# DomhnallBoyle/lip2speech-unit

Hardware: AMD Instinct MI355X
Metric: real-time factor (audio-sec/wall-sec), end-to-end lip->16kHz audio, 4s@25fps clips (higher is better)
Workload: dtype fp16; 1 GPU; e2e lip->units->wav (BASELINE configs[3]: AV-HuBERT large 24L + conformer 12x512 + multi_input HiFi-GAN), 4-s 100-frame 88x88 clips, batch 640 per GPU; clips_per_gpu=640, streams=1, clips_per_launch=640, frames_per_clip=100, hipgraph=True, input=uint8 96x96 frames resident in HBM, crop+normalise on device, enc_layers=24, conf_layers=12, parallelism=clip-parallel dp1

## Files before the change

include/lip2speech_hip.h:

```cpp
#ifndef LIP2SPEECH_HIP_H
#define LIP2SPEECH_HIP_H

#include <stddef.h>
#include <stdint.h>

#ifdef __cplusplus
extern "C" {
#endif

#define L2S_ABI_VERSION 16

enum { L2S_F16 = 0, L2S_BF16 = 1, L2S_F32 = 2 };

enum { L2S_OK = 0, L2S_EINVAL = -1, L2S_ESHAPE = -2, L2S_EALIGN = -3, L2S_EUNSUPPORTED = -4 };

enum {
  L2S_ACT_NONE = 0,
  L2S_ACT_RELU = 1,
  L2S_ACT_GELU = 2,
  L2S_ACT_SWISH = 3,
  L2S_ACT_PRELU = 4,
  L2S_ACT_LRELU = 5,
  L2S_ACT_TANH = 6
};
// ... 123 lines not shown
                              int B, int T, int C, int dtype, void* stream);
int l2s_lens_from_mask(const uint8_t* mask, int32_t* lens, int B, int T, void* stream);
int l2s_split_hi_lo(const float* x, int ldx, void* hi, void* lo, int ld16, int act, float slope, const int32_t* lens,
                    int len_mul, int B, int T, int C, int dtype, void* stream);

typedef struct l2s_respair_desc {
  const void* X; const void* W1; const void* W2; const float* b1; const float* b2;
  void* Y; float* XS; const int32_t* lens;
  int32_t len_mul, B, T, C, k, dil, last, accumulate, dtype;
  float slope;
} l2s_respair_desc;
int l2s_respair(const l2s_respair_desc* d, void* stream);
int l2s_respair_variant(const l2s_respair_desc* d);

typedef struct l2s_respair_final_desc {
  const void* X[3]; const void* W1[3]; const void* W2[3]; const float* b1[3]; const float* b2[3];
  int32_t k[3], dil[3];
  void* Y; const int32_t* lens;
  int32_t n, len_mul, B, T, C, dtype;
  float slope;
} l2s_respair_final_desc;
int l2s_respair_final(const l2s_respair_final_desc* d, void* stream);

int l2s_basicblock_fused(const void* x, const void* w1, const float* b1, const float* s1, const void* w2, const float* b2,
                         const float* s2, void* y, int n_images, int H, int W, int C, int dtype, void* stream);
int l2s_basiclayer_fused(const void* x, const void* const* w, const float* const* bias, const float* const* slope, int n_blocks,
                         void* y, int n_images, int H, int W, int C, int dtype, void* stream);
#define L2S_BB_PADDED64 576064
#define L2S_BB_PHASE64 512064
#define L2S_BB_PHASE128 256128
int l2s_basicblock_variant(int n_images, int H, int W, int C, int n_blocks, int dtype);
int l2s_basicstage128_tail_fused(const void* x0, const void* t0, const void* wa, const float* ba, const float* sa, const void* w1,
                                 const float* b1, const float* s1, const void* w2, const float* b2, const float* s2, void* y,
                                 int n_images, int H, int W, int dtype, void* stream);

int l2s_conv_post_tanh(const float* x, const float* w, float bias, float* wav, int16_t* pcm, const int32_t* lens,
                       int len_mul, int B, int T, int C, int k, void* stream);

int l2s_resblock_fused(const void* xl, const void* w, const float* bias, float* xs, void* xl_out,
                       const int32_t* lens, int len_mul, int B, int T, int C, int k, int d0, int d1, int d2,
                       int accumulate, float slope, int dtype, void* stream);

int l2s_resstage_fused(const void* xl, const void* const* w, const float* const* bias, const int* ks, const int* dils,
                       int n_blocks, float* xs, void* xl_out, const int32_t* lens, int len_mul, int B, int T, int C,
                       float slope, int xs_final, int dtype, void* stream);

// ... 106 lines not shown
```

lip2speech_unit_amd/_lib.py:

```python
import ctypes
import os

_HERE = os.path.dirname(os.path.abspath(__file__))
LIB_PATH = os.environ.get("L2S_LIB_PATH") or os.path.join(_HERE, "liblip2speech_hip.so")

F16, BF16, F32 = 0, 1, 2
ACT_NONE, ACT_RELU, ACT_GELU, ACT_SWISH, ACT_PRELU, ACT_LRELU, ACT_TANH = range(7)
F_RES_PRE, F_RES_POST, F_ACCUM, F_DUAL, F_MASK, F_OUT_F32, F_RES_F32 = (1 << i for i in range(7))
MODE_LINEAR, MODE_CONV1D, MODE_CONV2D = 0, 1, 2
ABI_VERSION = 16
SEQ_VARIANT_F32, LN_GENERIC, ATTN_RESIDENT = 2000, 10, 1000
BB_PADDED64, BB_PHASE64, BB_PHASE128 = 576064, 512064, 256128

_ERR = {-1: "L2S_EINVAL", -2: "L2S_ESHAPE", -3: "L2S_EALIGN", -4: "L2S_EUNSUPPORTED"}


class L2SError(RuntimeError):
    pass


class GemmDesc(ctypes.Structure):
    _fields_ = [
        ("A", ctypes.c_void_p), ("W", ctypes.c_void_p), ("C", ctypes.c_void_p), ("C2", ctypes.c_void_p),
        ("bias", ctypes.c_void_p), ("slope", ctypes.c_void_p), ("R", ctypes.c_void_p), ("lens", ctypes.c_void_p),
# ... 13 lines not shown
        ("ktab", ctypes.c_void_p),
    ]


_vp, _i, _f = ctypes.c_void_p, ctypes.c_int, ctypes.c_float


class RespairDesc(ctypes.Structure):
    _fields_ = [("X", ctypes.c_void_p), ("W1", ctypes.c_void_p), ("W2", ctypes.c_void_p), ("b1", ctypes.c_void_p),
                ("b2", ctypes.c_void_p), ("Y", ctypes.c_void_p), ("XS", ctypes.c_void_p), ("lens", ctypes.c_void_p),
                ("len_mul", ctypes.c_int32), ("B", ctypes.c_int32), ("T", ctypes.c_int32), ("C", ctypes.c_int32),
                ("k", ctypes.c_int32), ("dil", ctypes.c_int32), ("last", ctypes.c_int32), ("accumulate", ctypes.c_int32),
                ("dtype", ctypes.c_int32), ("slope", ctypes.c_float)]


class RespairFinalDesc(ctypes.Structure):
    _fields_ = [("X", ctypes.c_void_p * 3), ("W1", ctypes.c_void_p * 3), ("W2", ctypes.c_void_p * 3), ("b1", ctypes.c_void_p * 3),
                ("b2", ctypes.c_void_p * 3), ("k", ctypes.c_int32 * 3), ("dil", ctypes.c_int32 * 3),
                ("Y", ctypes.c_void_p), ("lens", ctypes.c_void_p),
                ("n", ctypes.c_int32), ("len_mul", ctypes.c_int32), ("B", ctypes.c_int32), ("T", ctypes.c_int32),
                ("C", ctypes.c_int32), ("dtype", ctypes.c_int32), ("slope", ctypes.c_float)]


SIGNATURES = {
    "l2s_abi_version": ([], ctypes.c_int),
    "l2s_build_info": ([], ctypes.c_char_p),
    "l2s_tapgemm": ([ctypes.POINTER(GemmDesc), _vp], _i),
    "l2s_tapgemm_variant": ([ctypes.POINTER(GemmDesc)], _i),
    "l2s_tapgemm_epilogue_family": ([ctypes.POINTER(GemmDesc)], _i),
    "l2s_stem_conv3d": ([_vp, _i, _vp, _vp, _vp, _vp, _i, _i, _i, _i, _i, _vp], _i),
    "l2s_stem_pool_fused": ([_vp, _i, _vp, _vp, _vp, _vp, _i, _i, _i, _i, _i, _vp], _i),
    "l2s_stem_pool_fused_u8": ([_vp, _i, _i, _i, _f, _f, _vp, _vp, _vp, _vp, _i, _i, _i, _vp], _i),
    "l2s_maxpool2d_3x3s2": ([_vp, _vp, _i, _i, _i, _i, _i, _vp], _i),
    "l2s_avgpool_hw": ([_vp, _vp, _i, _i, _i, _i, _vp], _i),
    "l2s_layernorm": ([_vp, _i, _i, _vp, _vp, _f, _vp, _i, _i, _vp, _i, _i, _i, _i, _vp, _i, _i, _i, _vp], _i),
    "l2s_layernorm_variant": ([_vp, _i, _i, _vp, _vp, _vp, _i, _i, _vp, _i, _i, _i, _i, _vp, _i, _i, _i], _i),
    "l2s_attention_variant": ([_vp, _i, _vp, _i, _vp, _i, _vp, _vp, _vp, _i, _i, _i, _i, _i], _i),
    "l2s_glu_dwconv_tile": ([_i, _i, _i, _i, _i], _i),
    "l2s_attention": ([_vp, _i, _vp, _i, _vp, _i, _vp, _vp, _vp, _i, _i, _i, _i, _i, _vp], _i),
    "l2s_glu_dwconv_swish": ([_vp, _vp, _vp, _vp, _vp, _i, _i, _i, _i, _i, _i, _vp], _i),
    "l2s_greedy_decode": ([_vp, _i, _vp, _i, _i, _i, _i, _f, _f, _vp, _vp, _vp, _vp], _i),
    "l2s_beam_decode": ([_vp, _i, _vp, _i, _i, _i, _i, _f, _f, _i, _vp, ctypes.c_size_t, _vp, _vp, _vp, _vp, _vp], _i),
    "l2s_beam_decode_workspace": ([_i, _i, _i], ctypes.c_size_t),
    "l2s_ctc_frames": ([_vp, _i, _vp, _i, _i, _i, _i, _i, _vp, _vp, _vp, _vp], _i),
    "l2s_ctc_beam_search": ([_vp, _vp, _vp, _i, _i, _i, _i, _i, _i, _vp, ctypes.c_size_t, _vp, _vp, _vp, _vp], _i),
    "l2s_ctc_beam_workspace": ([_i, _i, _i], ctypes.c_size_t),
# ... 1 lines not shown
    "l2s_repeat2_cast": ([_vp, _vp, _i, _i, _i, _i, _vp], _i),
    "l2s_splitk_reduce": ([_vp, _i, _i, _vp, _i, _i, _i, _vp], _i),
    "l2s_splitk_reduce_layernorm": ([_vp, _i, _i, _vp, _i, _vp, _vp, _f, _vp, _i, _i, _i, _i, _vp, _i, _i, _i, _vp], _i),
    "l2s_cast_f32_to_16": ([_vp, _i, _vp, _i, _i, _i, _i, _vp], _i),
    "l2s_cast_16_to_f32": ([_vp, _i, _vp, _i, _i, _i, _i, _vp], _i),
    "l2s_broadcast_rows": ([_vp, _i, _vp, _i, _i, _vp, _i, _i, _i, _i, _i, _i, _vp], _i),
    "l2s_transpose_ct_to_tc": ([_vp, _vp, _i, _i, _vp, _i, _i, _i, _i, _i, _vp], _i),
    "l2s_embedding": ([_vp, _vp, _vp, _i, _vp, _i, _i, _i, _i, _vp], _i),
    "l2s_embedding_tokens": ([_vp, _i, _i, _vp, _i, _vp, _i, _vp, _i, _i, _i, _i, _i, _vp], _i),
    "l2s_rows_f32_to_16_masked": ([_vp, _i, _vp, _i, _i, _vp, _i, _i, _i, _i, _i, _vp], _i),
    "l2s_lens_from_mask": ([_vp, _vp, _i, _i, _vp], _i),
    "l2s_basicblock_fused": ([_vp, _vp, _vp, _vp, _vp, _vp, _vp, _vp, _i, _i, _i, _i, _i, _vp], _i),
    "l2s_basiclayer_fused": ([_vp, _vp, _vp, _vp, _i, _vp, _i, _i, _i, _i, _i, _vp], _i),
    "l2s_basicblock_variant": ([_i, _i, _i, _i, _i, _i], _i),
    "l2s_stem_pool_frames": ([_i, _i], _i),
    "l2s_basicstage128_tail_fused": ([_vp] * 12 + [_i, _i, _i, _i, _vp], _i),
    "l2s_split_hi_lo": ([_vp, _i, _vp, _vp, _i, _i, _f, _vp, _i, _i, _i, _i, _i, _vp], _i),
    "l2s_conv_post_tanh": ([_vp, _vp, _f, _vp, _vp, _vp, _i, _i, _i, _i, _i, _vp], _i),
    "l2s_resblock_fused": ([_vp, _vp, _vp, _vp, _vp, _vp, _i, _i, _i, _i, _i, _i, _i, _i, _i, _f, _i, _vp], _i),
    "l2s_resstage_fused": ([_vp, _vp, _vp, _vp, _vp, _i, _vp, _vp, _vp, _i, _i, _i, _i, _f, _i, _i, _vp], _i),
    "l2s_respair": ([ctypes.POINTER(RespairDesc), _vp], _i),
    "l2s_respair_variant": ([ctypes.POINTER(RespairDesc)], _i),
    "l2s_respair_final": ([ctypes.POINTER(RespairFinalDesc), _vp], _i),
    "l2s_preprocess_frames": ([_vp, _vp, _i, _i, _i, _i, _i, _f, _f, _i, _vp], _i),
    "l2s_mel_spectrogram": ([_vp, _i, ctypes.c_int64, _vp, _i, _i, _vp, _vp, _vp, _vp, _i, _i, _i, _i, _i, _f, _vp], _i),
    "l2s_stft_mel": ([_vp, _i, ctypes.c_int64, _vp, _i, _i, _vp, _vp, _vp, _vp, _i, _i, _i, _i, _i, _i, _f, _f, _vp], _i),
    "l2s_unit_ce": ([_vp, _i, _vp, _i, _vp, _i, _i, _i, _i, _i, _i, _vp, _vp, _vp, _vp, _vp], _i),
    "l2s_mel_l1_sc": ([_vp, _i, _vp, _i, _vp, _i, _i, _i, _i, _vp, _vp, _vp, _vp, _vp], _i),
    "l2s_ctc_loss_workspace": ([_i, _i, _i], ctypes.c_size_t),
    "l2s_ctc_loss": ([_vp, _i, _vp, _i, _i, _i, _i, _i, _vp, _vp, _vp, _i, _vp, ctypes.c_size_t, _vp, _vp], _i),
    "l2s_wave_stem_workspace": ([_i, _i], ctypes.c_size_t),
    "l2s_wave_stem": ([_vp, _i, ctypes.c_int64, _vp, _i, _i, _vp, _vp, _vp, _f, _vp, _i, _i, _i, _vp, ctypes.c_size_t, _i, _vp], _i),
    "l2s_kmeans_assign": ([_vp, _i, _vp, _vp, _vp, _i, _i, _i, _i, _i, _vp, _vp, _vp], _i),
    "l2s_kmeans_nearest_workspace": ([_i], ctypes.c_size_t),
    "l2s_kmeans_nearest": ([_vp, _i, ctypes.c_int64, _vp, _i, _vp, _vp, _i, _i, _vp, _vp, _vp, _vp, ctypes.c_size_t, _vp], _i),
    "l2s_kmeans_update_workspace": ([_i, _i], ctypes.c_size_t),
    "l2s_kmeans_update": ([_vp, _i, ctypes.c_int64, _vp, _i, _vp, _vp, _vp, _i, _i, _vp, _vp, _vp, _vp, ctypes.c_size_t, _vp], _i),
    "l2s_kmeans_pp_workspace": ([_i], ctypes.c_size_t),
    "l2s_kmeans_pp_pot": ([_vp, _i, ctypes.c_int64, _vp, _i, _i, _vp, _i, _vp, _vp, _vp, _vp, _vp, _vp, ctypes.c_size_t, _vp], _i),
    "l2s_kmeans_pp_pick": ([_vp, _i, _vp, _i, _vp, _vp, _vp, _vp], _i),
    "l2s_stoi_resample": ([_vp, _i, ctypes.c_int64, _vp, _i, _i, _vp, _vp, ctypes.c_int64, _i, _vp], _i),
    "l2s_stoi_frames": ([_vp, ctypes.c_int64, _vp, _i, _i, _vp, _vp, _i, _vp, _vp], _i),
    "l2s_stoi_bands": ([_vp, _vp, ctypes.c_int64, _vp, _i, _i, _vp, _i, _vp, _vp, _vp, _vp, _vp, _i, _vp], _i),
    "l2s_stoi_scores": ([_vp, _i, _vp, _i, _vp, _i, _vp, _vp, _vp, _vp], _i),
    "l2s_wav_gain": ([_vp, _i, ctypes.c_int64, _vp, _i, _i, _f, _vp, _vp], _i),
    "l2s_stft_mel_power": ([_vp, _i, ctypes.c_int64, _vp, _vp, _vp, _i, _i, _vp, _vp, _vp, _vp, _i, _i, _i, _i, _i, _i, _vp], _i),
# ... 51 lines not shown
```

lip2speech_unit_amd/csrc/respair_phase.hip:

```cpp
#include "phase_stream.h"
#include "respair_args.h"
#include <cstdlib>

using namespace l2s;
using l2s_rp::RpArgs;

int l2s_respair_grid(int ntiles, int slots);

namespace {

constexpr int XT1 = 8;
constexpr int XRQ = 4;
template <int CH>
struct XGeo {
  static constexpr int NWC = CH / 64, NWR = 8 / NWC, NBLK = CH / 64;
  static constexpr int RM = NWR * 64;
  static constexpr int RPR = RM + 56;
  static constexpr int BLK_B = RPR * 128;
  static constexpr int REGION = NBLK * BLK_B;
  static constexpr int QROWS = NWC * 32;
  static constexpr int Q_B = QROWS * 128;
  static constexpr int DPW = QROWS >= 64 ? QROWS / 64 : 1;
  static constexpr int RPS = DPW * 8;
  static constexpr int BIAS_OFF = REGION + XRQ * Q_B;
// ... 166 lines not shown
    for (int i = 0; i < MI; ++i)
#pragma unroll
      for (int h = 0; h < 2; ++h) {
        const u32x4_t q = resp[i][h];
        const uint32_t w4[4] = {q.x, q.y, q.z, q.w};
#pragma unroll
        for (int e = 0; e < 8; ++e) {
          const float r = ET::to_f32((uint16_t)((w4[e >> 1] >> ((e & 1) * 16)) & 0xffff));
          acc[i][2 * h + (e >> 2)][e & 3] += fminf(r, r * inv_slope);
        }
      }
  }
  __device__ __forceinline__ void add_res(Acc& acc, const u32x2_t (&resq)[MI][NI], float inv_slope) const {
#pragma unroll
    for (int i = 0; i < MI; ++i)
#pragma unroll
      for (int j = 0; j < NI; ++j) {
        const float r[4] = {ET::to_f32((uint16_t)(resq[i][j].x & 0xffff)), ET::to_f32((uint16_t)(resq[i][j].x >> 16)),
                            ET::to_f32((uint16_t)(resq[i][j].y & 0xffff)), ET::to_f32((uint16_t)(resq[i][j].y >> 16))};
#pragma unroll
        for (int e = 0; e < 4; ++e) acc[i][j][e] += fminf(r[e], r[e] * inv_slope);
      }
  }
  __device__ __forceinline__ void write_t1(const Acc& acc, int g0, int len, float slope) const {
    u32x2_t t1v[MI][NI];
#pragma unroll
    for (int i = 0; i < MI; ++i) {
      const int t = g0 + wr * 64 + i * 16 + lm;
      const uint32_t km = (unsigned)t < (unsigned)len ? 0xffffffffu : 0u;
#pragma unroll
      for (int j = 0; j < NI; ++j) {
        f32x4_t v = acc[i][j];
        const f32x4_t sc = v * slope;
#pragma unroll
        for (int e = 0; e < 4; ++e) v[e] = fmaxf(v[e], sc[e]);
        t1v[i][j].x = ET::pack2(v[0], v[1]) & km;
        t1v[i][j].y = ET::pack2(v[2], v[3]) & km;
      }
    }
    __builtin_amdgcn_s_barrier();
    asm volatile("" ::: "memory");
#pragma unroll
    for (int i = 0; i < MI; ++i) {
      const int R = wr * 64 + i * 16 + lm + XT1;
      const uint32_t ta = lds_base + (uint32_t)wc * G::BLK_B + (uint32_t)R * 128;
      if constexpr (PAIRED) {
#pragma unroll
        for (int h = 0; h < 2; ++h)
          lds_write_u4(ta + (uint32_t)(((4 * h + lg) ^ (R & 7)) << 4),
                       u32x4_t{t1v[i][2 * h].x, t1v[i][2 * h].y, t1v[i][2 * h + 1].x, t1v[i][2 * h + 1].y});
      } else {
#pragma unroll
        for (int j = 0; j < NI; ++j) lds_write_u2(ta + (uint32_t)(((2 * j + (lg >> 1)) ^ (R & 7)) << 4) + (uint32_t)((lg & 1) * 8), t1v[i][j]);
      }
    }
  }
  __device__ __forceinline__ static int64_t out_row(int r, int unit, int g0, int halo, int T) {
    const int t = g0 + r;
    return (r >= halo && r < G::RM - halo && t < T) ? (int64_t)unit * T + t : (int64_t)-1;
  }
  __device__ __forceinline__ void store_y(uint16_t* Y, Acc& acc, int unit, int g0, int halo, int T, int len, float slope) const {
    auto rowmap = [&](int r) -> int64_t { return out_row(r, unit, g0, halo, T); };
    l2s_gemm_desc p = {};
    p.C = Y; p.bias = nullptr; p.N = CH; p.ldc = CH; p.act = L2S_ACT_LRELU; p.act_slope = slope; p.alpha = 1.f;
    p.mask_T = T; p.mask_mul = 1;
    int ln = lane;
    asm volatile("" : "+v"(ln));
    epilogue_direct16<ET, MI, NI, L2S_EPI_F16 + 3, decltype(rowmap), NoHook, true>(p, acc, ln, wr * 64, wc * 64, 0, rowmap, unit * T, len);
  }
};

template <typename ET, int CH, int KIND>
__global__ __launch_bounds__(512) void respair_phase_kernel(const RpArgs a) {
  using G = XGeo<CH>;
  constexpr int MI = 4, NI = 4;
  constexpr bool PAIRED = KIND == 0;
  extern __shared__ __attribute__((aligned(16))) uint16_t lds[];
  const int tid = threadIdx.x;
  const TileWalk tiles(a.ntiles, a.xcd_order);
// ... 203 lines not shown
      pc.barrier_then_stagger();
      pc.template run_conv<0>(acc1, k, dil, h2, stage_one);

      pc.level();
      {
        u32x4_t resp[MI][2];
        pc.read_res(resp, h1);
        pc.add_res(sum, resp, inv_slope);
      }
      pc.write_t1(acc1, g0, len, slope);
      asm volatile("s_waitcnt lgkmcnt(0)" ::: "memory");
      pc.barrier_then_stagger();
      pc.template run_conv<1>(sum, k, dil, h2, stage_one);

      pc.level();
      if (j + 1 < nj) issue_patch(c_i, j + 1);
      else if (c_i + 1 < tiles.n) issue_patch(c_i + 1, 0);
    }
    pc.store_y(a.Y, sum, unit, g0, h2max, T, len, slope);
  }
  wait_vmcnt<0>();
}

template <typename ET, int CH>
int launch_respair_final(const l2s_rp::RpFinalArgs& a, hipStream_t st) {
  using G = XGeo<CH>;
  constexpr int SMEM = G::BIAS_OFF + 4 * CH * 4;
  static_assert(SMEM <= 160 * 1024, "LDS");
  auto kern = respair_final_kernel<ET, CH>;
  static L2sSmemOptIn opt_in;
  if (int e = l2s_smem_opt_in(kern, SMEM, opt_in)) return e;
  const int grid = l2s_respair_grid(a.ntiles, 256);
  hipLaunchKernelGGL(kern, dim3(grid), dim3(512), SMEM, st, a);
  L2S_CHECK_LAUNCH();
  return L2S_OK;
}

template <typename ET, int CH, int KIND>
int launch_respair_phase(const RpArgs& a, hipStream_t st) {
  using G = XGeo<CH>;
  auto kern = respair_phase_kernel<ET, CH, KIND>;
  static L2sSmemOptIn opt_in;
  if (int e = l2s_smem_opt_in(kern, G::SMEM, opt_in)) return e;
  const int grid = l2s_respair_grid(a.ntiles, 256);
  hipLaunchKernelGGL(kern, dim3(grid), dim3(512), G::SMEM, st, a);
  L2S_CHECK_LAUNCH();
// ... 44 lines not shown
    a.X[j] = (const uint16_t*)d->X[j]; a.W1[j] = (const uint16_t*)d->W1[j]; a.W2[j] = (const uint16_t*)d->W2[j];
    a.b1[j] = d->b1[j]; a.b2[j] = d->b2[j]; a.k[j] = d->k[j]; a.dil[j] = d->dil[j];
    h2max = h2 > h2max ? h2 : h2max;
  }
  for (int j = d->n; j < 3; ++j) { a.X[j] = a.X[0]; a.W1[j] = a.W1[0]; a.W2[j] = a.W2[0]; a.b1[j] = a.b1[0]; a.b2[j] = a.b2[0]; a.k[j] = a.k[0]; a.dil[j] = a.dil[0]; }
  if ((uintptr_t)d->Y & 15) return L2S_EALIGN;
  a.Y = (uint16_t*)d->Y; a.lens = d->lens; a.nj = d->n; a.len_mul = d->len_mul; a.T = d->T; a.h2max = h2max;
  a.S = l2s_respair_phase_rows(d->C) - 2 * h2max;
  a.tiles_per_clip = (d->T + a.S - 1) / a.S;
  a.ntiles = d->B * a.tiles_per_clip;
  a.xcd_order = 1;
  a.slope = d->slope;
  hipStream_t st = (hipStream_t)stream;
  auto go = [&](auto et) -> int {
    using ET = decltype(et);
    if (d->C == 256) return launch_respair_final<ET, 256>(a, st);
    if (d->C == 128) return launch_respair_final<ET, 128>(a, st);
    return launch_respair_final<ET, 64>(a, st);
  };
  if (d->dtype == L2S_F16) return go(ElemF16{});
  if (d->dtype == L2S_BF16) return go(ElemBF16{});
  return L2S_EINVAL;
}
```

lip2speech_unit_amd/ops.py:

```python
import ctypes
import os
from typing import Optional

import torch

from . import _lib
from ._lib import (ACT_GELU, ACT_LRELU, ACT_NONE, ACT_PRELU, ACT_RELU, ACT_SWISH, ACT_TANH, BF16, F16, F32, F_ACCUM,
                   F_DUAL, F_MASK, F_OUT_F32, F_RES_F32, F_RES_POST, F_RES_PRE, MODE_CONV1D, MODE_CONV2D,
                   MODE_LINEAR, GemmDesc, L2SError, check)

_TORCH16 = {F16: torch.float16, BF16: torch.bfloat16, F32: torch.float32}
_DTYPE_NAME = {F16: "f16", BF16: "bf16", F32: "f32"}


class KernelProfiler:

    def __init__(self, detail=False):
        self.records = []
        self.detail = detail

    def summary(self):
        torch.cuda.synchronize()
        agg = {}
        for key, fl, by, e0, e1, shape in self.records:
# ... 442 lines not shown
    d.lens = fake if lens else None
    d.len_mul, d.B, d.T, d.C, d.k, d.dil = len_mul, B, T, C, k, dil
    d.last, d.accumulate, d.dtype, d.slope = last, int(bool(accumulate)), dtype, float(slope)
    return _lib.load().l2s_respair_variant(ctypes.byref(d))


def respair_final(xs_l, w1s, b1s, w2s, b2s, y, *, B, T, C, ks, dils, slope, lens=None, len_mul=1, dtype=F16):
    lib = _lib.load()
    n = len(xs_l)
    if not (1 <= n <= 3 and len(w1s) == len(w2s) == len(b1s) == len(b2s) == len(ks) == len(dils) == n):
        raise L2SError("respair_final: 1..3 ResBlocks, one entry per list each")
    d = _lib.RespairFinalDesc()
    for j in range(n):
        d.X[j], d.W1[j], d.W2[j] = _ptr(_req(xs_l[j], _TORCH16[dtype], "x_l")), _ptr(w1s[j]), _ptr(w2s[j])
        d.b1[j], d.b2[j] = _ptr(_req(b1s[j], torch.float32, "b1")), _ptr(_req(b2s[j], torch.float32, "b2"))
        d.k[j], d.dil[j] = int(ks[j]), int(dils[j])
    if lens is not None and lens.dtype != torch.int32:
        raise L2SError("lens must be int32")
    d.Y, d.lens = _ptr(_req(y, _TORCH16[dtype], "y")), _ptr(lens)
    d.n, d.len_mul, d.B, d.T, d.C, d.dtype, d.slope = n, len_mul, B, T, C, dtype, float(slope)
    _run(f"l2s_respair_final<C{C}>", lambda: lib.l2s_respair_final(ctypes.byref(d), _stream()),
         flops=sum(2.0 * B * T * C * C * k * 2 for k in ks), nbytes=float(B) * T * C * 2 * (n + 1) + sum(2.0 * 2 * C * C * k for k in ks),
         shape=f"M{B * T} n{n}")


def preprocess_frames(frames, y, *, B, T, Hin, Win, crop=88, mean=0.421, std=0.165, dtype=F16):
    _run("l2s_preprocess_frames", lambda: _lib.load().l2s_preprocess_frames(_ptr(frames), _ptr(y), B, T, Hin, Win, crop, mean, std, dtype, _stream()))


def mel_spectrogram(wav, mel, basis, fb, fb_range, *, B, S, T_rows, n_samples=None, ldw=None, ldm=None, n_fft=640, hop=160, n_mels=80,
                    floor=1e-5):
    if wav.dtype not in (torch.float32, torch.int16):
        raise L2SError(f"wav: expected float32 or int16, got {wav.dtype}")
    if n_samples is not None and n_samples.dtype != torch.int32:
        raise L2SError("n_samples must be int32")
    _req(wav, None, "wav"), _req(mel, torch.float32, "mel"), _req(basis, torch.float32, "basis"), _req(fb, torch.float32, "fb")
    _req(fb_range, torch.int32, "fb_range")
    frames = float(B) * T_rows
    _run("l2s_mel_spectrogram", lambda: _lib.load().l2s_mel_spectrogram(
        _ptr(wav), int(wav.dtype == torch.int16), ldw if ldw is not None else S, _ptr(n_samples), B, S, _ptr(basis), _ptr(fb),
        _ptr(fb_range), _ptr(mel), ldm if ldm is not None else n_mels, T_rows, n_fft, hop, n_mels, float(floor), _stream()),
        flops=2.0 * frames * n_fft * n_fft, nbytes=float(B) * S * wav.element_size() + 4.0 * frames * n_mels + 4.0 * n_fft * n_fft)


def stft_mel(wav, mel, basis, fb, fb_range, *, B, S, T_rows, n_fft, hop, pad, mag_eps=0.0, n_samples=None, ldw=None, ldm=None, n_mels=80,
             floor=1e-5):
# ... 752 lines not shown
                      "int len_mul=1, int dtype=0) -> ()",
    "transpose_ct_to_tc": "(Tensor x, Tensor(a!) y, *, int B, int C, int T, int ldy, int col0=0, Tensor? lens=None, int len_mul=1, "
                          "int dtype=0) -> ()",
    "embedding": "(Tensor code, Tensor table, Tensor(a!) y, *, int B, int L, int C, int? ldy=None, Tensor? lens=None, int dtype=0) -> ()",
    "embedding_tokens": "(Tensor tok, Tensor table, Tensor(a!) y, *, int B, int L, int C, int token_offset=4, int? ldt=None, "
                        "int? ldy=None, Tensor? lens=None, int len_mul=1, int dtype=0) -> ()",
    "rows_f32_to_16_masked": "(Tensor x, Tensor(a!) y, *, int B, int T, int C, int? ldx=None, int? ldy=None, int col0=0, "
                             "Tensor? lens=None, int len_mul=1, int dtype=0) -> ()",
    "lens_from_mask": "(Tensor? padding_mask, int B, int T, Device device) -> Tensor",
    "basicblock_fused": "(Tensor x, Tensor w1, Tensor b1, Tensor s1, Tensor w2, Tensor b2, Tensor s2, Tensor(a!) y, *, int n_images, "
                        "int H, int W, int C=64, int dtype=0) -> ()",
    "basiclayer_fused": _BL,
    "basicstage128_tail_fused": "(Tensor x0, Tensor t0, Tensor wa, Tensor ba, Tensor sa, Tensor w1, Tensor b1, Tensor s1, Tensor w2, "
                                "Tensor b2, Tensor s2, Tensor(a!) y, *, int n_images, int H, int W, int dtype=0) -> ()",
    "split_hi_lo": "(Tensor x, Tensor(a!) hi, Tensor(b!) lo, *, int B, int T, int C, int act=0, float slope=0.0, int? ldx=None, "
                   "int? ld16=None, Tensor? lens=None, int len_mul=1, int dtype=0) -> ()",
    "conv_post_tanh": _CPT,
    "resblock_fused": "(Tensor xl, Tensor w, Tensor bias, Tensor(a!) xs, Tensor(b!)? xl_out, *, int B, int T, int C, int k, int[] dil, "
                      "bool accumulate, float slope, Tensor? lens=None, int len_mul=1, int dtype=0) -> ()",
    "resstage_fused": "(Tensor xl, Tensor[] ws, Tensor[] biases, Tensor(a!) xs, Tensor(b!)? xl_out, *, int B, int T, int C, int[] ks, "
                      "int[] dils, float slope, Tensor? lens=None, int len_mul=1, int dtype=0, bool xs_final=True) -> ()",
    "respair": _RP,
    "respair_final": "(Tensor[] xs_l, Tensor[] w1s, Tensor[] b1s, Tensor[] w2s, Tensor[] b2s, Tensor(a!) y, *, int B, int T, int C, int[] ks, "
                     "int[] dils, float slope, Tensor? lens=None, int len_mul=1, int dtype=0) -> ()",
    "preprocess_frames": "(Tensor frames, Tensor(a!) y, *, int B, int T, int Hin, int Win, int crop=88, float mean=0.421, "
                         "float std=0.165, int dtype=0) -> ()",
    "mel_spectrogram": "(Tensor wav, Tensor(a!) mel, Tensor basis, Tensor fb, Tensor fb_range, *, int B, int S, int T_rows, "
                       "Tensor? n_samples=None, int? ldw=None, int? ldm=None, int n_fft=640, int hop=160, int n_mels=80, "
                       "float floor=1e-05) -> ()",
    "stft_mel": "(Tensor wav, Tensor(a!) mel, Tensor basis, Tensor fb, Tensor fb_range, *, int B, int S, int T_rows, int n_fft, int hop, "
                "int pad, float mag_eps=0.0, Tensor? n_samples=None, int? ldw=None, int? ldm=None, int n_mels=80, "
                "float floor=1e-05) -> ()",
    "unit_ce": "(Tensor logits, Tensor target, Tensor(a!) nll, Tensor(b!) smooth, Tensor(c!) n_correct, Tensor(d!) n_tok, *, int B, "
               "int T2, int V, int? ldl=None, int? ldt=None, Tensor? lens=None, int len_mul=2, int pad_idx=1, "
               "int ignore_prefix=0) -> ()",
    "mel_l1_sc": "(Tensor pred, Tensor targ, Tensor(a!) l1, Tensor(b!) sq, Tensor(c!) tsq, Tensor(d!) n_rows, *, int B, int Tm_pred, "
                 "int Tm_targ, int crop_len, Tensor? lens=None, int len_mul=4, int n_mels=80) -> ()",
    "ctc_loss": "(Tensor logits, Tensor targets, Tensor tgt_lens, Tensor tgt_offs, Tensor(a!) workspace, Tensor(b!) nll, *, int B, "
                "int L, int V, int S_max, int blank=0, int? ldl=None, Tensor? lens=None, int len_mul=2) -> ()",
    "wave_stem": "(Tensor wav, Tensor w, Tensor gamma, Tensor beta, Tensor(a!) workspace, Tensor(b!) out, *, int B, int S, int T_rows, "
                 "int C=512, Tensor? n_samples=None, int? ldw=None, int? ldo=None, float eps=1e-05, int dtype=0) -> ()",
    "kmeans_assign": "(Tensor x, Tensor centers, Tensor cnorm, Tensor(a!) ids, *, int B, int T, int D, int K, int? ldx=None, "
                     "Tensor? lens=None, int len_mul=1, Tensor(b!)? best2=None) -> ()",
    "kmeans_nearest": "(Tensor x, Tensor centers, Tensor cnorm, *, int M, int D, int K, Tensor? rows=None, Tensor(a!)? ids=None, "
                      "Tensor(b!)? dmin=None, Tensor(c!)? inertia=None, Tensor(d!)? workspace=None, int? ldx=None) -> ()",
    "kmeans_update": "(Tensor x, Tensor ids, Tensor centers, Tensor counts, Tensor(a!) centers_out, Tensor(b!) counts_out, "
# ... 32 lines not shown
                    "Tensor? suppress=None, Tensor? begin_suppress=None, Tensor? step=None, int first_step=0, "
                    "Tensor(d!)? logits=None, int? ldx=None, int? lde=None, int dtype=0) -> ()",
    "whisper_advance": "(Tensor(a!) token, Tensor logprob, Tensor(b!) tokens, Tensor(c!) sum_logprob, Tensor(d!) lengths, "
                       "Tensor(e!) done, Tensor tok_emb, Tensor pos_emb, Tensor(f!) x_next, Tensor(g!) pos, Tensor(h!) n_active, *, "
                       "int B, int V, int d, int eot, int? lde=None, int? ldx=None, int dtype=0) -> ()",
    "beam_attention": "(Tensor q, Tensor(a!) k_cache, Tensor(b!) v_cache, Tensor(c!) out, *, int B, int beam, int H, int hd, "
                      "Tensor? k_new=None, Tensor? v_new=None, Tensor? anc=None, Tensor? step=None, Tensor? enc_lens=None, "
                      "Tensor? n_live=None, Tensor? finished=None, int? ldq=None, int? ld_new=None, int? ldo=None, int dtype=0) -> ()",
    "beam_select": "(Tensor logits, Tensor scores, Tensor step, Tensor max_len, Tensor(a!) cand_score, Tensor(b!) cand_slot, "
                   "Tensor(c!) cand_token, *, int B, int beam, int V, int pad, int unk, int eos, int min_len=1, float temperature=1.0, "
                   "float unk_penalty=0.0, Tensor? n_live=None, Tensor? finished=None, int? ldl=None) -> ()",
    "beam_advance": "(Tensor cand_score, Tensor cand_slot, Tensor cand_token, Tensor(a!) tokens, Tensor(b!) anc, Tensor(c!) scores, "
                    "Tensor(d!) n_live, Tensor(e!) finished, Tensor(f!) parents, Tensor(g!) hyp_tokens, Tensor(h!) hyp_len, "
                    "Tensor(i!) hyp_score, Tensor(j!) nhyp, Tensor(k!) out_tokens, Tensor(l!) out_len, Tensor(m!) out_score, "
                    "Tensor max_len, Tensor emb, Tensor pos_table, Tensor(n!) x_next, Tensor(o!) step, Tensor(p!) n_active, *, int B, "
                    "int beam, int V, int d, int eos, int pad, float embed_scale=1.0, float lenpen=1.0, bool normalize_scores=True, "
                    "int? lde=None, int? ldx=None, int dtype=0) -> ()",
    "logfbank": "(Tensor wav, Tensor(a!) out, Tensor basis, Tensor fb, Tensor fb_range, *, int B, int S, int T_rows, int stack=4, "
                "bool normalize=True, Tensor? n_samples=None, Tensor? n_rows=None, int? ldw=None, int? ldo=None) -> ()",
}
ENTRY_OF = {n: "l2s_" + n for n in _SCHEMAS}
ENTRY_OF.update({"maxpool2d_3x3s2": "l2s_maxpool2d_3x3s2", "avgpool_hw": "l2s_avgpool_hw"})
HOST_QUERIES = ("l2s_abi_version", "l2s_build_info", "l2s_tapgemm_variant", "l2s_tapgemm_epilogue_family", "l2s_attention_variant", "l2s_layernorm_variant", "l2s_respair_variant",
                "l2s_glu_dwconv_tile", "l2s_basicblock_variant", "l2s_stem_pool_frames", "l2s_beam_decode_workspace",
                "l2s_ctc_beam_workspace", "l2s_ctc_loss_workspace", "l2s_wave_stem_workspace", "l2s_kmeans_nearest_workspace",
                "l2s_kmeans_update_workspace", "l2s_kmeans_pp_workspace", "l2s_vocab_argmax_workspace", "l2s_whisper_logmel_workspace",
                "l2s_beam_select_workspace")
ALIASES = {"frontend3d_stem": "stem_pool_fused", "resnet_trunk": "basiclayer_fused", "linear_epilogue": "tapgemm",
           "posconv_gelu": "tapgemm", "convtranspose1d": "tapgemm", "mel_head": "tapgemm", "mhsa_padmask": "attention",
           "relpos_mhsa": "attention", "conformer_conv_module": "glu_dwconv_swish", "greedy_unit_decode": "greedy_decode",
           "resblock1": "respair", "tanh_to_int16": "conv_post_tanh"}

_TORCH_LIB = torch.library.Library("lip2speech", "DEF")


def _fake_none(*a, **k):
    return None


def _fake_beam_decode(logits, *, B, T2, V, beam, ldl=None, lens=None, len_mul=1, temperature=1.0, lenpen=1.0):
    return (logits.new_empty((B, beam, T2 + 1), dtype=torch.int32), logits.new_empty((B, beam, T2 + 1), dtype=torch.float32),
            logits.new_empty((B, beam), dtype=torch.float32), logits.new_empty((B,), dtype=torch.int32))


def _fake_lens_from_mask(padding_mask, B, T, device):
    return torch.empty(B, device=device, dtype=torch.int32)
# ... 52 lines not shown
```

lip2speech_unit_amd/vocoder.py:

```python
import os

import torch
import torch.nn as nn

from . import ops
from .ops import ACT_GELU, ACT_LRELU, F_ACCUM, F_DUAL, F_MASK, F_RES_POST, MODE_CONV1D
from .packing import PackedState, convtranspose_fused, convtranspose_phases, pack_conv1d

LRELU_SLOPE = 0.1
FUSED_PAIR = os.environ.get("L2S_RESPAIR", "1") != "0"
FUSED_PAIR256 = os.environ.get("L2S_RESPAIR256", "1") != "0"
PAIR_MIN_TILES = int(os.environ.get("L2S_RESPAIR_MIN_TILES", "64"))
PAIR_ROWS = {256: 128, 128: 256, 64: 512}
FUSED_UPS = os.environ.get("L2S_FUSED_UPS", "1") != "0"
FUSED_UPS_MAX_CIN = int(os.environ.get("L2S_FUSED_UPS_MAX_CIN", "128"))
FUSED_STAGE = os.environ.get("L2S_RESSTAGE", "1") != "0"
FUSED_FINAL = os.environ.get("L2S_RESPAIR_FINAL", "1") != "0"
SKIP_DEAD_XS = os.environ.get("L2S_SKIP_DEAD_XS", "1") != "0"


class AttrDict(dict):

    def __init__(self, *args, **kwargs):
        super().__init__(*args, **kwargs)
        self.__dict__ = self


def get_padding(kernel_size, dilation=1):
    return int((kernel_size * dilation - dilation) / 2)


class _WN(nn.Module):

    def __init__(self, shape, bias_n, g_dim0):
        super().__init__()
        self.weight_g = nn.Parameter(torch.ones(g_dim0, 1, 1))
        self.weight_v = nn.Parameter(torch.zeros(*shape))
        self.bias = nn.Parameter(torch.zeros(bias_n))

    def effective_weight(self):
        if hasattr(self, "weight") and isinstance(getattr(self, "weight"), torch.Tensor):
# ... 197 lines not shown
                            act_slope=LRELU_SLOPE, lens=lens, mask_T=T // fd, mask_mul=mul // u // fd, flags=F_MASK, dtype=dt)
            elif pair_stage or fused_stage:
                x = None
                for ph in st["phases"]:
                    ops.tapgemm(x_l, ph["w"], xl, M=M_in, N=C, Cin=st["cin"], ntaps=ph["ntaps"], mode=MODE_CONV1D, T_out=T,
                                T_in=T, stride=1, dil=-1, off=ph["off"], out_row_mul=u, out_row_add=ph["r"], bias=st["b"],
                                act=ACT_LRELU, act_slope=LRELU_SLOPE, lens=lens, mask_T=To, mask_mul=mul, flags=F_MASK,
                                dtype=dt)
            else:
                x = torch.empty(M, C, device=dev, dtype=t16)
                for ph in st["phases"]:
                    ops.tapgemm(x_l, ph["w"], x, M=M_in, N=C, Cin=st["cin"], ntaps=ph["ntaps"], mode=MODE_CONV1D, T_out=T,
                                T_in=T, stride=1, dil=-1, off=ph["off"], out_row_mul=u, out_row_add=ph["r"], bias=st["b"],
                                C2=xl, ldc2=C, lens=lens, mask_T=To, mask_mul=mul, flags=F_DUAL | F_MASK,
                                slope2=LRELU_SLOPE, dtype=dt)
            nxt = torch.empty(M, C, device=dev, dtype=t16)
            last_stage = si == len(P["stages"]) - 1
            final_fused = pair_stage and FUSED_FINAL and SKIP_DEAD_XS and not last_stage and len(st["rbs"]) <= 3
            xs = None if final_fused else torch.empty(M, C, device=dev, dtype=torch.float32)
            if pair_stage:
                finals = []
                for j, rb in enumerate(st["rbs"]):
                    cur_l = xl
                    for m, cv in enumerate(rb["convs"]):
                        if final_fused and m == len(rb["convs"]) - 1:
                            finals.append((cur_l, cv, rb["k"]))
                        elif m < len(rb["convs"]) - 1:
                            ol = torch.empty(M, C, device=dev, dtype=t16)
                            ops.respair(cur_l, cv["w1"], cv["b1"], cv["w2"], cv["b2"], B=B, T=To, C=C, k=rb["k"], dil=cv["d"],
                                        slope=LRELU_SLOPE, y=ol, lens=lens, len_mul=mul, dtype=dt)
                            cur_l = ol
                        else:
                            dual = (j == len(st["rbs"]) - 1) and not last_stage
                            ops.respair(cur_l, cv["w1"], cv["b1"], cv["w2"], cv["b2"], B=B, T=To, C=C, k=rb["k"], dil=cv["d"],
                                        slope=LRELU_SLOPE, xs=xs, y=nxt if dual else None, accumulate=j > 0, lens=lens,
                                        len_mul=mul, dtype=dt, xs_final=not (dual and SKIP_DEAD_XS))
                if finals:
                    ops.respair_final([f[0] for f in finals], [f[1]["w1"] for f in finals], [f[1]["b1"] for f in finals],
                                      [f[1]["w2"] for f in finals], [f[1]["b2"] for f in finals], nxt, B=B, T=To, C=C,
                                      ks=[f[2] for f in finals], dils=[f[1]["d"] for f in finals], slope=LRELU_SLOPE, lens=lens,
                                      len_mul=mul, dtype=dt)
                x_l, T = nxt, To
                continue
            if fused_stage:
                if FUSED_STAGE and [rb["k"] for rb in st["rbs"]] == [3, 7, 11]:
                    ops.resstage_fused(xl, [rb["fw"] for rb in st["rbs"]], [rb["fb"] for rb in st["rbs"]], xs,
                                       None if last_stage else nxt, B=B, T=To, C=C, ks=[rb["k"] for rb in st["rbs"]],
# ... 296 lines not shown
```

Before: 13330 audio-sec/wall-sec.

## Chain two consecutive HiFi-GAN residual conv pairs in one LDS-resident kernel

Adds a respair_chain kernel that runs the first two dilated conv pairs of a three-conv resblock back to back on one tile. The intermediate activation stays in LDS instead of going through HBM, and one kernel launch replaces two. It is used for C=128 with k=3 and for C=64 with k=3 or 7, when the tile count is high enough. The cost is a larger combined halo: fewer useful rows per tile and extra recomputed rows at tile edges.

Measured after the change: 13380 audio-sec/wall-sec (median of 6 runs). Within noise of the previous version (+0.4%).

```diff
diff --git a/include/lip2speech_hip.h b/include/lip2speech_hip.h
--- a/include/lip2speech_hip.h
+++ b/include/lip2speech_hip.h
@@ -169,6 +169,15 @@
 } l2s_respair_final_desc;
 int l2s_respair_final(const l2s_respair_final_desc* d, void* stream);
 
+typedef struct l2s_respair_chain_desc {
+  const void* X; const void* W1[2]; const void* W2[2]; const float* b1[2]; const float* b2[2];
+  void* Y; const int32_t* lens;
+  int32_t len_mul, B, T, C, k, dil[2], dtype;
+  float slope;
+} l2s_respair_chain_desc;
+int l2s_respair_chain(const l2s_respair_chain_desc* d, void* stream);
+int l2s_respair_chain_variant(const l2s_respair_chain_desc* d);
+
 int l2s_basicblock_fused(const void* x, const void* w1, const float* b1, const float* s1, const void* w2, const float* b2,
                          const float* s2, void* y, int n_images, int H, int W, int C, int dtype, void* stream);
 int l2s_basiclayer_fused(const void* x, const void* const* w, const float* const* bias, const float* const* slope, int n_blocks,
diff --git a/lip2speech_unit_amd/_lib.py b/lip2speech_unit_amd/_lib.py
--- a/lip2speech_unit_amd/_lib.py
+++ b/lip2speech_unit_amd/_lib.py
@@ -59,6 +59,13 @@
                 ("C", ctypes.c_int32), ("dtype", ctypes.c_int32), ("slope", ctypes.c_float)]
 
 
+class RespairChainDesc(ctypes.Structure):
+    _fields_ = [("X", ctypes.c_void_p), ("W1", ctypes.c_void_p * 2), ("W2", ctypes.c_void_p * 2), ("b1", ctypes.c_void_p * 2),
+                ("b2", ctypes.c_void_p * 2), ("Y", ctypes.c_void_p), ("lens", ctypes.c_void_p),
+                ("len_mul", ctypes.c_int32), ("B", ctypes.c_int32), ("T", ctypes.c_int32), ("C", ctypes.c_int32),
+                ("k", ctypes.c_int32), ("dil", ctypes.c_int32 * 2), ("dtype", ctypes.c_int32), ("slope", ctypes.c_float)]
+
+
 SIGNATURES = {
     "l2s_abi_version": ([], ctypes.c_int),
     "l2s_build_info": ([], ctypes.c_char_p),
@@ -106,6 +113,8 @@
     "l2s_respair": ([ctypes.POINTER(RespairDesc), _vp], _i),
     "l2s_respair_variant": ([ctypes.POINTER(RespairDesc)], _i),
     "l2s_respair_final": ([ctypes.POINTER(RespairFinalDesc), _vp], _i),
+    "l2s_respair_chain": ([ctypes.POINTER(RespairChainDesc), _vp], _i),
+    "l2s_respair_chain_variant": ([ctypes.POINTER(RespairChainDesc)], _i),
     "l2s_preprocess_frames": ([_vp, _vp, _i, _i, _i, _i, _i, _f, _f, _i, _vp], _i),
     "l2s_mel_spectrogram": ([_vp, _i, ctypes.c_int64, _vp, _i, _i, _vp, _vp, _vp, _vp, _i, _i, _i, _i, _i, _f, _vp], _i),
     "l2s_stft_mel": ([_vp, _i, ctypes.c_int64, _vp, _i, _i, _vp, _vp, _vp, _vp, _i, _i, _i, _i, _i, _i, _f, _f, _vp], _i),
diff --git a/lip2speech_unit_amd/csrc/respair_phase.hip b/lip2speech_unit_amd/csrc/respair_phase.hip
--- a/lip2speech_unit_amd/csrc/respair_phase.hip
+++ b/lip2speech_unit_amd/csrc/respair_phase.hip
@@ -212,7 +212,8 @@
         for (int e = 0; e < 4; ++e) acc[i][j][e] += fminf(r[e], r[e] * inv_slope);
       }
   }
-  __device__ __forceinline__ void write_t1(const Acc& acc, int g0, int len, float slope) const {
+  template <bool BARRIER>
+  __device__ __forceinline__ void write_rows(const Acc& acc, int g0, int len, float slope, int row0) const {
     u32x2_t t1v[MI][NI];
 #pragma unroll
     for (int i = 0; i < MI; ++i) {
@@ -228,11 +229,13 @@
         t1v[i][j].y = ET::pack2(v[2], v[3]) & km;
       }
     }
-    __builtin_amdgcn_s_barrier();
-    asm volatile("" ::: "memory");
+    if constexpr (BARRIER) {
+      __builtin_amdgcn_s_barrier();
+      asm volatile("" ::: "memory");
+    }
 #pragma unroll
     for (int i = 0; i < MI; ++i) {
-      const int R = wr * 64 + i * 16 + lm + XT1;
+      const int R = wr * 64 + i * 16 + lm + row0;
       const uint32_t ta = lds_base + (uint32_t)wc * G::BLK_B + (uint32_t)R * 128;
       if constexpr (PAIRED) {
 #pragma unroll
@@ -245,6 +248,7 @@
       }
     }
   }
+  __device__ __forceinline__ void write_t1(const Acc& acc, int g0, int len, float slope) const { write_rows<true>(acc, g0, len, slope, XT1); }
   __device__ __forceinline__ static int64_t out_row(int r, int unit, int g0, int halo, int T) {
     const int t = g0 + r;
     return (r >= halo && r < G::RM - halo && t < T) ? (int64_t)unit * T + t : (int64_t)-1;
@@ -494,6 +498,117 @@
   wait_vmcnt<0>();
 }
 
+struct RpChainArgs {
+  const uint16_t* X; const uint16_t* W[4]; const float* b[4];
+  uint16_t* Y; const int32_t* lens;
+  int len_mul, T, k, dil[2], halo, S, ntiles, tiles_per_clip, xcd_order;
+  float slope;
+};
+
+template <typename ET, int CH>
+__global__ __launch_bounds__(512) void respair_chain_kernel(const RpChainArgs a) {
+  using G = XGeo<CH>;
+  constexpr int MI = 4, NI = 4;
+  extern __shared__ __attribute__((aligned(16))) uint16_t lds[];
+  const int tid = threadIdx.x;
+  const TileWalk tiles(a.ntiles, a.xcd_order);
+  if (tiles.n <= 0) return;
+  PairCore<ET, CH, true> pc(lds, tid);
+  const int k = a.k, h2 = (k - 1) / 2, T = a.T, halo = a.halo;
+  const int h1A = h2 * a.dil[0], h1B = h2 * a.dil[1];
+  const int nkt = k * G::NBLK;
+
+  uint32_t w_lane[G::DPW];
+  pc.lane_offsets(w_lane, k);
+  const uint32_t h_bytes = (uint32_t)(32 * k * CH) * 2u;
+  const char* kt_ptr = (const char*)a.W[0];
+  int s_kt = 0, s_conv = 0;
+  auto stage_one = [&](auto dslot_tag, auto sh_tag) {
+    constexpr int DSLOT = decltype(dslot_tag)::value, SH = decltype(sh_tag)::value;
+    pc.template stage_quarter<DSLOT>(kt_ptr + (size_t)(SH ? h_bytes : 0u), w_lane);
+    if constexpr (SH == 1) {
+      kt_ptr += 128;
+      if (++s_kt == nkt) {
+        s_kt = 0;
+        s_conv = (s_conv + 1) & 3;
+        kt_ptr = (const char*)(s_conv == 0 ? a.W[0] : (s_conv == 1 ? a.W[1] : (s_conv == 2 ? a.W[2] : a.W[3])));
+      }
+    }
+  };
+
+  f32x4_t acc[MI][NI];
+  for (int i = tid; i < 4 * CH; i += 512) {
+    const int j = i / CH, c = i - j * CH;
+    reinterpret_cast<float*>(lds)[G::BIAS_OFF / 4 + i] = (j == 0 ? a.b[0] : (j == 1 ? a.b[1] : (j == 2 ? a.b[2] : a.b[3])))[c];
+  }
+  __syncthreads();
+  const float slope = a.slope, inv_slope = 1.0f / a.slope;
+  pc.init_acc(acc, 0);
+
+  auto issue_patch = [&](int i) {
+    int unit, g0;
+    tiles.origin(i, a.tiles_per_clip, a.S, halo, unit, g0);
+    pc.issue_patch(a.X, unit, g0, h1A, T);
+  };
+  issue_patch(0);
+  stage_one(std::integral_constant<int, 0>{}, std::integral_constant<int, 0>{});
+  stage_one(std::integral_constant<int, 1>{}, std::integral_constant<int, 1>{});
+  for (int c_i = 0; c_i < tiles.n; ++c_i) {
+    int unit, g0;
+    tiles.origin(c_i, a.tiles_per_clip, a.S, halo, unit, g0);
+    int len = a.lens ? a.lens[unit] * a.len_mul : T;
+    len = len < T ? len : T;
+    wait_vmcnt<0>();
+#pragma unroll
+    for (int p = 0; p < 2; ++p) {
+      const int dil = p ? a.dil[1] : a.dil[0], h1 = p ? h1B : h1A;
+      pc.barrier_then_stagger();
+      pc.template run_conv<0>(acc, k, dil, h2, stage_one);
+
+      pc.level();
+      u32x4_t res[MI][2];
+      pc.read_res(res, h1);
+      pc.write_t1(acc, g0, len, slope);
+      pc.init_acc(acc, 2 * p + 1);
+      asm volatile("s_waitcnt lgkmcnt(0)" ::: "memory");
+      pc.barrier_then_stagger();
+      pc.template run_conv<1>(acc, k, dil, h2, stage_one);
+
+      pc.level();
+      if (p == 0) {
+        pc.add_res(acc, res, inv_slope);
+#pragma unroll
+        for (int i = 0; i < MI; ++i)
+#pragma unroll
+          for (int j = 0; j < NI; ++j) acc[i][j] = acc[i][j] + 0.f;
+        pc.template write_rows<false>(acc, g0, len, slope, h1B);
+        pc.init_acc(acc, 2);
+        asm volatile("s_waitcnt lgkmcnt(0)" ::: "memory");
+      } else {
+        if (c_i + 1 < tiles.n) issue_patch(c_i + 1);
+        pc.add_res(acc, res, inv_slope);
+        pc.store_y(a.Y, acc, unit, g0, halo, T, len, slope);
+        pc.init_acc(acc, 0);
+      }
+    }
+  }
+  wait_vmcnt<0>();
+}
+
+template <typename ET, int CH>
+int launch_respair_chain(const RpChainArgs& a, hipStream_t st) {
+  using G = XGeo<CH>;
+  constexpr int SMEM = G::BIAS_OFF + 4 * CH * 4;
+  static_assert(SMEM <= 160 * 1024, "LDS");
+  auto kern = respair_chain_kernel<ET, CH>;
+  static L2sSmemOptIn opt_in;
+  if (int e = l2s_smem_opt_in(kern, SMEM, opt_in)) return e;
+  const int grid = l2s_respair_grid(a.ntiles, 256);
+  hipLaunchKernelGGL(kern, dim3(grid), dim3(512), SMEM, st, a);
+  L2S_CHECK_LAUNCH();
+  return L2S_OK;
+}
+
 template <typename ET, int CH>
 int launch_respair_final(const l2s_rp::RpFinalArgs& a, hipStream_t st) {
   using G = XGeo<CH>;
@@ -584,3 +699,62 @@
   if (d->dtype == L2S_BF16) return go(ElemBF16{});
   return L2S_EINVAL;
 }
+
+bool l2s_respair_chain_supports(int C, int kA, int dA, int kB, int dB) {
+  if (kA != kB || kA < 1 || !(kA & 1) || dA < 1 || dB < 1 || dA > 1000 || dB > 1000 || kA > 2001) return false;
+  const int h2 = (kA - 1) / 2, h1A = h2 * dA, h1B = h2 * dB;
+  if (!l2s_respair_phase_supports(C, h1A, h2) || !l2s_respair_phase_supports(C, h1B, h2)) return false;
+  const int rm = l2s_respair_phase_rows(C), H = h1A + h2 + h1B + h2;
+  return 2 * H <= 56 && rm - 2 * H >= rm / 2;
+}
+
+namespace {
+
+int respair_chain_select(const l2s_respair_chain_desc* d) {
+  if (!d || !d->X || !d->Y) return L2S_EINVAL;
+  for (int p = 0; p < 2; ++p)
+    if (!d->W1[p] || !d->W2[p] || !d->b1[p] || !d->b2[p]) return L2S_EINVAL;
+  if (d->B <= 0 || d->T <= 0 || d->k < 1 || !(d->k & 1) || d->dil[0] < 1 || d->dil[1] < 1) return L2S_ESHAPE;
+  if (d->C != 64 && d->C != 128 && d->C != 256) return L2S_EUNSUPPORTED;
+  if (!l2s_respair_chain_supports(d->C, d->k, d->dil[0], d->k, d->dil[1])) return L2S_EUNSUPPORTED;
+  if (!(d->slope > 0.f && d->slope <= 1.f) || (d->lens && d->len_mul <= 0)) return L2S_EINVAL;
+  if (((uintptr_t)d->X & 15) || ((uintptr_t)d->Y & 15)) return L2S_EALIGN;
+  for (int p = 0; p < 2; ++p)
+    if (((uintptr_t)d->W1[p] & 15) || ((uintptr_t)d->W2[p] & 15) || ((uintptr_t)d->b1[p] & 15) || ((uintptr_t)d->b2[p] & 15)) return L2S_EALIGN;
+  if ((int64_t)d->B * d->T >= ((int64_t)1 << 31) / 2) return L2S_EUNSUPPORTED;
+  if (d->dtype != L2S_F16 && d->dtype != L2S_BF16) return L2S_EINVAL;
+  return l2s_respair_phase_rows(d->C) * 1000 + d->C;
+}
+
+}
+
+extern "C" int l2s_respair_chain_variant(const l2s_respair_chain_desc* d) { return respair_chain_select(d); }
+
+extern "C" int l2s_respair_chain(const l2s_respair_chain_desc* d, void* stream) {
+  const int variant = respair_chain_select(d);
+  if (variant < 0) return variant;
+  const int h2 = (d->k - 1) / 2;
+  RpChainArgs a = {};
+  a.X = (const uint16_t*)d->X;
+  for (int p = 0; p < 2; ++p) {
+    a.W[2 * p] = (const uint16_t*)d->W1[p]; a.W[2 * p + 1] = (const uint16_t*)d->W2[p];
+    a.b[2 * p] = d->b1[p]; a.b[2 * p + 1] = d->b2[p];
+    a.dil[p] = d->dil[p];
+  }
+  a.Y = (uint16_t*)d->Y; a.lens = d->lens; a.len_mul = d->len_mul; a.T = d->T; a.k = d->k;
+  a.halo = h2 * d->dil[0] + h2 + h2 * d->dil[1] + h2;
+  a.S = variant / 1000 - 2 * a.halo;
+  a.tiles_per_clip = (d->T + a.S - 1) / a.S;
+  a.ntiles = d->B * a.tiles_per_clip;
+  static const int xcd_on = [] { const char* e = getenv("L2S_RESPAIR_XCD"); return e ? atoi(e) : 1; }();
+  a.xcd_order = xcd_on;
+  a.slope = d->slope;
+  hipStream_t st = (hipStream_t)stream;
+  auto go = [&](auto et) -> int {
+    using ET = decltype(et);
+    if (d->C == 256) return launch_respair_chain<ET, 256>(a, st);
+    if (d->C == 128) return launch_respair_chain<ET, 128>(a, st);
+    return launch_respair_chain<ET, 64>(a, st);
+  };
+  return d->dtype == L2S_F16 ? go(ElemF16{}) : go(ElemBF16{});
+}
diff --git a/lip2speech_unit_amd/ops.py b/lip2speech_unit_amd/ops.py
--- a/lip2speech_unit_amd/ops.py
+++ b/lip2speech_unit_amd/ops.py
@@ -488,6 +488,38 @@
     _run(f"l2s_respair_final<C{C}>", lambda: lib.l2s_respair_final(ctypes.byref(d), _stream()),
          flops=sum(2.0 * B * T * C * C * k * 2 for k in ks), nbytes=float(B) * T * C * 2 * (n + 1) + sum(2.0 * 2 * C * C * k for k in ks),
          shape=f"M{B * T} n{n}")
+
+
+def respair_chain(x_l, w1s, b1s, w2s, b2s, y, *, B, T, C, k, dils, slope, lens=None, len_mul=1, dtype=F16):
+    lib = _lib.load()
+    if not (len(w1s) == len(w2s) == len(b1s) == len(b2s) == len(dils) == 2):
+        raise L2SError("respair_chain: two pairs, one entry per list each")
+    d = _lib.RespairChainDesc()
+    for p in range(2):
+        d.W1[p], d.W2[p] = _ptr(w1s[p]), _ptr(w2s[p])
+        d.b1[p], d.b2[p] = _ptr(_req(b1s[p], torch.float32, "b1")), _ptr(_req(b2s[p], torch.float32, "b2"))
+        d.dil[p] = int(dils[p])
+    if lens is not None and lens.dtype != torch.int32:
+        raise L2SError("lens must be int32")
+    d.X, d.Y, d.lens = _ptr(_req(x_l, _TORCH16[dtype], "x_l")), _ptr(_req(y, _TORCH16[dtype], "y")), _ptr(lens)
+    d.len_mul, d.B, d.T, d.C, d.k, d.dtype, d.slope = len_mul, B, T, C, k, dtype, float(slope)
+    key = f"l2s_respair_chain<C{C}>"
+    if _profiler is not None and _profiler.detail:
+        key += f" k{k} dil{dils[0]}-{dils[1]}"
+    _run(key, lambda: lib.l2s_respair_chain(ctypes.byref(d), _stream()),
+         flops=2 * 2.0 * B * T * C * C * k * 2, nbytes=float(B) * T * C * 2 * 2 + 2 * 2.0 * 2 * C * C * k, shape=f"M{B * T} k{k}")
+
+
+def respair_chain_variant(*, B, T, C, k, dils, slope=0.1, lens=True, len_mul=1, dtype=F16):
+    d = _lib.RespairChainDesc()
+    fake = 0x10000
+    d.X = d.Y = fake
+    for p in range(2):
+        d.W1[p] = d.W2[p] = d.b1[p] = d.b2[p] = fake
+        d.dil[p] = int(dils[p])
+    d.lens = fake if lens else None
+    d.len_mul, d.B, d.T, d.C, d.k, d.dtype, d.slope = len_mul, B, T, C, k, dtype, float(slope)
+    return _lib.load().l2s_respair_chain_variant(ctypes.byref(d))
 
 
 def preprocess_frames(frames, y, *, B, T, Hin, Win, crop=88, mean=0.421, std=0.165, dtype=F16):
@@ -1286,6 +1318,8 @@
                       "int[] dils, float slope, Tensor? lens=None, int len_mul=1, int dtype=0, bool xs_final=True) -> ()",
     "respair": _RP,
     "respair_final": "(Tensor[] xs_l, Tensor[] w1s, Tensor[] b1s, Tensor[] w2s, Tensor[] b2s, Tensor(a!) y, *, int B, int T, int C, int[] ks, "
+                     "int[] dils, float slope, Tensor? lens=None, int len_mul=1, int dtype=0) -> ()",
+    "respair_chain": "(Tensor x_l, Tensor[] w1s, Tensor[] b1s, Tensor[] w2s, Tensor[] b2s, Tensor(a!) y, *, int B, int T, int C, int k, "
                      "int[] dils, float slope, Tensor? lens=None, int len_mul=1, int dtype=0) -> ()",
     "preprocess_frames": "(Tensor frames, Tensor(a!) y, *, int B, int T, int Hin, int Win, int crop=88, float mean=0.421, "
                          "float std=0.165, int dtype=0) -> ()",
@@ -1364,6 +1398,7 @@
 ENTRY_OF = {n: "l2s_" + n for n in _SCHEMAS}
 ENTRY_OF.update({"maxpool2d_3x3s2": "l2s_maxpool2d_3x3s2", "avgpool_hw": "l2s_avgpool_hw"})
 HOST_QUERIES = ("l2s_abi_version", "l2s_build_info", "l2s_tapgemm_variant", "l2s_tapgemm_epilogue_family", "l2s_attention_variant", "l2s_layernorm_variant", "l2s_respair_variant",
+                "l2s_respair_chain_variant",
                 "l2s_glu_dwconv_tile", "l2s_basicblock_variant", "l2s_stem_pool_frames", "l2s_beam_decode_workspace",
                 "l2s_ctc_beam_workspace", "l2s_ctc_loss_workspace", "l2s_wave_stem_workspace", "l2s_kmeans_nearest_workspace",
                 "l2s_kmeans_update_workspace", "l2s_kmeans_pp_workspace", "l2s_vocab_argmax_workspace", "l2s_whisper_logmel_workspace",
diff --git a/lip2speech_unit_amd/vocoder.py b/lip2speech_unit_amd/vocoder.py
--- a/lip2speech_unit_amd/vocoder.py
+++ b/lip2speech_unit_amd/vocoder.py
@@ -16,7 +16,19 @@
 FUSED_UPS_MAX_CIN = int(os.environ.get("L2S_FUSED_UPS_MAX_CIN", "128"))
 FUSED_STAGE = os.environ.get("L2S_RESSTAGE", "1") != "0"
 FUSED_FINAL = os.environ.get("L2S_RESPAIR_FINAL", "1") != "0"
+PAIR_CHAIN = os.environ.get("L2S_RESPAIR_CHAIN", "1") != "0"
+CHAIN_K = {256: (), 128: (3,), 64: (3, 7)}
 SKIP_DEAD_XS = os.environ.get("L2S_SKIP_DEAD_XS", "1") != "0"
+
+
+def _chain_taken(rb, B, To, C, mul, dt):
+    if not (PAIR_CHAIN and len(rb["convs"]) == 3 and rb["k"] in CHAIN_K.get(C, ())):
+        return False
+    k, dils = rb["k"], [rb["convs"][0]["d"], rb["convs"][1]["d"]]
+    if ops.respair_chain_variant(B=B, T=To, C=C, k=k, dils=dils, slope=LRELU_SLOPE, len_mul=mul, dtype=dt) < 0:
+        return False
+    S = PAIR_ROWS[C] - (k - 1) * (2 + dils[0] + dils[1])
+    return B * -(-To // S) >= PAIR_MIN_TILES
 
 
 class AttrDict(dict):
@@ -260,7 +272,17 @@
                 finals = []
                 for j, rb in enumerate(st["rbs"]):
                     cur_l = xl
+                    chained = _chain_taken(rb, B, To, C, mul, dt)
+                    if chained:
+                        ca, cb = rb["convs"][0], rb["convs"][1]
+                        ol = torch.empty(M, C, device=dev, dtype=t16)
+                        ops.respair_chain(cur_l, [ca["w1"], cb["w1"]], [ca["b1"], cb["b1"]], [ca["w2"], cb["w2"]], [ca["b2"], cb["b2"]],
+                                          ol, B=B, T=To, C=C, k=rb["k"], dils=[ca["d"], cb["d"]], slope=LRELU_SLOPE, lens=lens,
+                                          len_mul=mul, dtype=dt)
+                        cur_l = ol
                     for m, cv in enumerate(rb["convs"]):
+                        if chained and m < 2:
+                            continue
                         if final_fused and m == len(rb["convs"]) - 1:
                             finals.append((cur_l, cv, rb["k"]))
                         elif m < len(rb["convs"]) - 1:
```
